# krrish94/nerf-pytorch

Hardware: AMD Instinct MI355X
Metric: train rays/sec (higher is better)
Workload: dtype f32

## Files before the change

### include/nerfhip.h

```cpp
#ifndef NERFHIP_H_
#define NERFHIP_H_

#include <stddef.h>
#include <stdint.h>

#ifdef __cplusplus
extern "C" {
#endif

typedef void* nerfhip_stream_t;

#define NERFHIP_OK 0
#define NERFHIP_ERR_ARG (-1)
#define NERFHIP_ERR_UNSUPPORTED (-2)
#define NERFHIP_ERR_LAUNCH (-3)
#define NERFHIP_ERR_WORKSPACE (-4)

#define NERFHIP_RNG_UNIFORM 0
#define NERFHIP_RNG_NORMAL 1

int nerfhip_version(void);
const char* nerfhip_last_error(void);
int nerfhip_is_emulated(void);

// ... 75 lines not shown
int nerfhip_plan_dim_xyz(nerfhip_plan_t plan);
int nerfhip_plan_dim_dir(nerfhip_plan_t plan);
int nerfhip_plan_num_tensors(nerfhip_plan_t plan);
int nerfhip_plan_tensor_info(nerfhip_plan_t plan, int i, const char** name, int64_t* offset, int* rows, int* cols);
int nerfhip_plan_describe(nerfhip_plan_t plan, char* buf, int64_t cap);
int64_t nerfhip_plan_packed_floats(nerfhip_plan_t plan);
int nerfhip_plan_pack_index(nerfhip_plan_t plan, int32_t* host_table);
int nerfhip_pack_weights(const float* params, const int32_t* table, int64_t n, float* packed, nerfhip_stream_t stream);
int nerfhip_pack_weights_plan(nerfhip_plan_t plan, const float* params, const int32_t* table, float* packed,
                              nerfhip_stream_t stream);
int64_t nerfhip_plan_stash_bytes(nerfhip_plan_t plan, int64_t m);
int64_t nerfhip_plan_bwd_scratch_bytes(nerfhip_plan_t plan, int64_t m);
int nerfhip_plan_set_bwd_compaction(nerfhip_plan_t plan, int on);
int nerfhip_plan_bwd_compaction(nerfhip_plan_t plan);
int64_t nerfhip_plan_bwd_stats_offset(nerfhip_plan_t plan, int64_t m);
int nerfhip_plan_set_freqs(nerfhip_plan_t plan, const float* freqs_xyz, const float* freqs_dir);

int nerfhip_mlp_fwd(nerfhip_plan_t plan, const float* packed, const float* x, int64_t m, float* out, void* stash,
                    nerfhip_stream_t stream);
int nerfhip_mlp_bwd(nerfhip_plan_t plan, const float* packed, const float* g_out, int64_t m, const void* stash,
                    void* scratch, int64_t scratch_bytes, float* g_params, nerfhip_stream_t stream);
int nerfhip_mlp_bwd_input(nerfhip_plan_t plan, const float* params, int64_t m, const void* scratch, float* g_x,
                          nerfhip_stream_t stream);

typedef struct nerfhip_render_cfg {
    int num_coarse;
    int num_fine;
    int perturb;
    int lindisp;
    int white_background;
// ... 250 lines not shown
```

### nerf-pytorch_amd/_lib.py

```python
import ctypes as C
import os

_HERE = os.path.dirname(os.path.abspath(__file__))
LIB_PATH = os.path.join(_HERE, "libnerfhip.so")

c_f = C.c_void_p
c_i64 = C.c_int64
c_u64 = C.c_uint64
c_u32 = C.c_uint32


class ModelCfg(C.Structure):
    _fields_ = [(n, C.c_int) for n in (
        "num_layers", "hidden_size", "skip_connect_every", "num_encoding_fn_xyz", "num_encoding_fn_dir",
        "include_input_xyz", "include_input_dir", "log_sampling_xyz", "log_sampling_dir", "use_viewdirs")]


class RenderCfg(C.Structure):
    _fields_ = [("num_coarse", C.c_int), ("num_fine", C.c_int), ("perturb", C.c_int), ("lindisp", C.c_int),
                ("white_background", C.c_int), ("noise_std", C.c_float), ("ray_stride", C.c_int)]


class RenderRand(C.Structure):
    _fields_ = [("t_rand", c_f), ("noise_coarse", c_f), ("u", c_f), ("noise_fine", c_f)]
# ... 72 lines not shown
    "nerfhip_plan_dim_xyz": (C.c_int, [C.c_void_p]),
    "nerfhip_plan_dim_dir": (C.c_int, [C.c_void_p]),
    "nerfhip_plan_num_tensors": (C.c_int, [C.c_void_p]),
    "nerfhip_plan_tensor_info": (C.c_int, [C.c_void_p, C.c_int, C.POINTER(C.c_char_p), C.POINTER(c_i64),
                                            C.POINTER(C.c_int), C.POINTER(C.c_int)]),
    "nerfhip_plan_packed_floats": (c_i64, [C.c_void_p]),
    "nerfhip_plan_describe": (C.c_int, [C.c_void_p, C.c_char_p, c_i64]),
    "nerfhip_plan_pack_index": (C.c_int, [C.c_void_p, C.c_void_p]),
    "nerfhip_pack_weights": (C.c_int, [c_f, c_f, c_i64, c_f, c_f]),
    "nerfhip_plan_stash_bytes": (c_i64, [C.c_void_p, c_i64]),
    "nerfhip_plan_bwd_scratch_bytes": (c_i64, [C.c_void_p, c_i64]),
    "nerfhip_plan_set_freqs": (C.c_int, [C.c_void_p, C.c_void_p, C.c_void_p]),
    "nerfhip_plan_set_bwd_compaction": (C.c_int, [C.c_void_p, C.c_int]),
    "nerfhip_plan_bwd_compaction": (C.c_int, [C.c_void_p]),
    "nerfhip_plan_bwd_stats_offset": (c_i64, [C.c_void_p, c_i64]),
    "nerfhip_mlp_fwd": (C.c_int, [C.c_void_p, c_f, c_f, c_i64, c_f, c_f, c_f]),
    "nerfhip_mlp_bwd": (C.c_int, [C.c_void_p, c_f, c_f, c_i64, c_f, c_f, c_i64, c_f, c_f]),
    "nerfhip_mlp_bwd_input": (C.c_int, [C.c_void_p, c_f, c_i64, c_f, c_f, c_f]),
    "nerfhip_render_workspace_bytes": (c_i64, [C.c_void_p, C.c_void_p, C.POINTER(RenderCfg), c_i64, C.c_int]),
    "nerfhip_render_workspace_region": (C.c_int, [C.c_void_p, C.c_void_p, C.POINTER(RenderCfg), c_i64, C.c_int, C.c_char_p,
                                                   C.POINTER(c_i64), C.POINTER(c_i64)]),
    "nerfhip_render_fwd": (C.c_int, [C.c_void_p, C.c_void_p, C.POINTER(RenderCfg), c_f, c_i64, c_f, c_f, c_f, c_f,
                                      C.POINTER(RenderRand), c_u64, c_u64, C.POINTER(RenderOut), c_f, c_i64, C.c_int,
                                      c_f]),
    "nerfhip_render_bwd": (C.c_int, [C.c_void_p, C.c_void_p, C.POINTER(RenderCfg), c_f, c_i64, c_f, c_f,
                                      C.POINTER(RenderRand), c_u64, c_u64, c_f, c_f, c_f, c_i64, c_f, c_f, c_f]),
    "nerfhip_render_fwd_parts": (C.c_int, [C.c_void_p, C.c_void_p, C.POINTER(RenderCfg), c_f, c_i64, c_f, c_f, c_f, c_f,
                                            C.POINTER(RenderRand), c_u64, c_u64, C.POINTER(RenderOut), c_f, c_i64,
                                            C.c_int, C.c_int, c_f]),
    "nerfhip_render_bwd_parts": (C.c_int, [C.c_void_p, C.c_void_p, C.POINTER(RenderCfg), c_f, c_i64, c_f, c_f,
# ... 163 lines not shown
```

### nerf-pytorch_amd/csrc/wgrad_f16.hip

```cpp
#include <vector>

#include "nh_device.h"
#include "nh_diag.h"
#include "nh_mlp.h"

namespace {

constexpr int NHW_MAX_JOBS = 40;
#ifndef NHW_WAVES
#define NHW_WAVES 8
#endif
constexpr int NHW_THREADS = 64 * NHW_WAVES;
#ifndef NHW_STAGES
#define NHW_STAGES 2
#endif

struct WgBJob {
    int64_t a_off, b_off;
    int wg0, nwg;
    int r_hi, col_count, w_ld;
    int64_t w_off, bias_off;
    int a_idx, b_idx;
    int64_t s_w_off;
    int s_w_ld;
};
struct WgBArgs {
    const float* stash;
    const float* grad;
    float* partial;
    float* g_params;
    int64_t nt;
    int njobs, part_stride;
    const unsigned* amax;
    const unsigned* bmax;
    int64_t s_off, s_bias_off;
    int s_idx, s_r_lo, s_r_hi, s_col_base, s_col_count;
    signed char scol[64];
    const int* cidx;
    const int* cstats;
    WgBJob jobs[NHW_MAX_JOBS];
};

NH_DEVICE int region_shift(unsigned word) { return word <= 1u ? 0 : 14 - ((int)word - 256); }
NH_DEVICE float unscale2(float v, int sa, int sb) { return (v * nh_pow2i(-sa)) * nh_pow2i(-sb); }

template <int AR, int BR, int SA = 0, int SB = 0>
struct WShape {
    static_assert(SA == 0 || SB == 0, "one guest per block");
    static_assert(NHW_WAVES == 8, "the side tiles are dealt to a 4 x 2 wave grid");
    static constexpr int PO = AR / (16 * NHW_WAVES), PI = BR / 64, TA = AR / 32, TB = BR / 32;
    static constexpr int SR = SA + SB;
    static constexpr int STAGE_A = AR * 64, STAGE_B = BR * 64, STAGE_S = SR * 64;
    static constexpr int STAGE = STAGE_A + STAGE_B + STAGE_S;
    static constexpr int OPER_A = AR * 32, OPER_B = BR * 32, OPER_S = SR * 32;
    static constexpr int LDS_BYTES = NHW_STAGES * STAGE + 2 * (OPER_A + OPER_B + OPER_S);
    static constexpr int SIDE_TILES = SB ? TA * (SB / 32) : (SA ? TB : 0);
    static constexpr int PART = AR * BR + SIDE_TILES * 1024 + NHW_THREADS + (SA ? 64 : 0);
};

template <int ROWS>
struct RowItems {
    static constexpr int N = (ROWS * 2 + NHW_THREADS - 1) / NHW_THREADS;
    float v[N][8];
};
template <int ROWS>
NH_DEVICE void rows_load(const float* stage, int tid, RowItems<ROWS>& r) {
#pragma unroll
    for (int it = 0; it < RowItems<ROWS>::N; ++it) {
        const int id = tid + NHW_THREADS * it;
        const bool on = ROWS * 2 % NHW_THREADS == 0 || id < ROWS * 2;
        const int row = id % ROWS, q = on ? id / ROWS : 0;
#pragma unroll
        for (int e = 0; e < 8; ++e) r.v[it][e] = on ? stage[(8 * q + e) * ROWS + row] : 0.0f;
    }
}
template <int ROWS>
NH_DEVICE float rows_store(const RowItems<ROWS>& r, char* hi_blocks, char* lo_blocks, int tid, float scale) {
    float sum = 0.0f;
#pragma unroll
    for (int it = 0; it < RowItems<ROWS>::N; ++it) {
        const int id = tid + NHW_THREADS * it;
        if (ROWS * 2 % NHW_THREADS != 0 && id >= ROWS * 2) break;
        const int row = id % ROWS, q = id / ROWS;
        nh_f16x8 h8, l8;
#pragma unroll
        for (int e = 0; e < 8; ++e) {
            float v = r.v[it][e];
            sum += v;
#ifdef NHW_EXP_NO_CONVERT
            h8[e] = nh_to_f16(v);
            l8[e] = h8[e];
            continue;
#endif
            v *= scale;
            const nh_f16 hi = nh_to_f16(v);
            h8[e] = hi;
            l8[e] = nh_to_f16(v - nh_from_f16(hi));
        }
        const int off = (((row >> 5) * 2 + q) * 32 + (row & 31)) * 16;
        *(nh_f16x8*)(hi_blocks + off) = h8;
        *(nh_f16x8*)(lo_blocks + off) = l8;
    }
    return sum;
// ... 17 lines not shown
        nh_dma16a(src, lane * 16, (int)(rows[0] * (unsigned)RB + ((unsigned)p * 1024u) % RB), lds_dst);
    } else {
        const int e = (lane * 16) / RB;
        unsigned row = rows[0];
#pragma unroll
        for (int k = 1; k < N; ++k) {
            row = e == k ? rows[k] : row;
#ifndef NERFHIP_EMU
            asm volatile("" : "+v"(row));
#endif
        }
        nh_dma16a(src, (int)(row * (unsigned)RB + (unsigned)(lane * 16) % RB), 0, lds_dst);
    }
}

template <int AR, int BR, int SA = 0, int SB = 0, bool CX = false>
NH_KERNEL void NH_LB(NHW_THREADS, NHW_WAVES / 4) k_wgrad_f16x3(WgBArgs a) {
    using S = WShape<AR, BR, SA, SB>;
    constexpr int PO = S::PO, PI = S::PI, SR = S::SR;
    NH_DYN_LDS(lds);
    char* const ah_blk = lds + NHW_STAGES * S::STAGE;
    char* const al_blk = ah_blk + S::OPER_A;
    char* const bh_blk = al_blk + S::OPER_A;
    char* const bl_blk = bh_blk + S::OPER_B;
    char* const sh_blk = bl_blk + S::OPER_B;
    char* const sl_blk = sh_blk + S::OPER_S;
    const int lane = nh_lane(), wave = nh_wave_in_block(), tid = (int)threadIdx.x;
    int jq = 0;
    while (jq + 1 < a.njobs && (int)blockIdx.x >= a.jobs[jq + 1].wg0) ++jq;
    const WgBJob& jb = a.jobs[jq];
    const int64_t k = (int64_t)blockIdx.x - jb.wg0;
    const int64_t ntl = CX ? (int64_t)((nh_uload_i32(a.cstats, NH_CSTAT_ACTIVE) + 31) >> 5) : a.nt;
    const int64_t u0 = 2 * (ntl * k / jb.nwg), u1 = 2 * (ntl * (k + 1) / jb.nwg);
    const float* const a_reg = a.grad + jb.a_off;
    const float* const b_reg = a.stash + jb.b_off;
    const float* const s_reg = SR ? (SA ? a.grad : a.stash) + a.s_off : nullptr;
    const float a_scale = a.amax ? nh_pow2i(region_shift(a.amax[jb.a_idx])) : 1.0f;
    const float b_scale = a.bmax ? nh_pow2i(region_shift(a.bmax[jb.b_idx])) : 1.0f;
    const float s_scale = (SR && a.amax && a.bmax) ? nh_pow2i(region_shift((SA ? a.amax : a.bmax)[a.s_idx])) : 1.0f;
    const unsigned lds0 = nh_lds_addr((const float*)lds);
    constexpr int PIECES = (S::STAGE_A + S::STAGE_B) / (1024 * NHW_WAVES);
    constexpr int SPIECES = S::STAGE_S / 1024;
    static_assert(S::STAGE_A % (1024 * NHW_WAVES) == 0 && S::STAGE_B % (1024 * NHW_WAVES) == 0, "every wave issues the same number of pieces");
    static_assert(SPIECES <= NHW_WAVES, "at most one side piece per wave");
    constexpr int NPB = S::STAGE_B / 1024 / NHW_WAVES;
    static_assert(!CX || NPB * NHW_WAVES * 1024 == S::STAGE_B, "every wave gathers the same number of B pieces");
    unsigned rb[NPB * GatherN<BR>::N > 0 ? NPB * GatherN<BR>::N : 1], rs[GatherN<(SB ? SB : 32)>::N];
    auto preload = [&](int64_t u) {
        if (CX && a.cidx) {
#pragma unroll
            for (int j = 0; j < NPB; ++j) gather_rows<BR>(rb + j * GatherN<BR>::N, a.cidx, (int)u * 16, wave + j * NHW_WAVES);
            if (SB) gather_rows<(SB ? SB : 32)>(rs, a.cidx, (int)u * 16, wave < SPIECES ? wave : 0);
        }
    };
    auto issue = [&](int64_t u) {
        const NhDmaSrc da = nh_dma_src(a_reg + (size_t)u * 16 * AR, (unsigned)S::STAGE_A);
        const unsigned st = lds0 + (unsigned)((int)(u % NHW_STAGES) * S::STAGE);
        for (int p = wave; p < S::STAGE_A / 1024; p += NHW_WAVES) nh_dma16a(da, lane * 16, p * 1024, st + (unsigned)(p * 1024));
        if (CX && a.cidx) {
            const NhDmaSrc db = nh_dma_src(b_reg, (unsigned)((size_t)a.nt * 32 * BR * 4));
#pragma unroll
            for (int j = 0; j < NPB; ++j)
                gather_piece_f16<BR>(db, rb + j * GatherN<BR>::N, wave + j * NHW_WAVES, lane, st + (unsigned)(S::STAGE_A + (wave + j * NHW_WAVES) * 1024));
        } else {
            const NhDmaSrc db = nh_dma_src(b_reg + (size_t)u * 16 * BR, (unsigned)S::STAGE_B);
            for (int p = wave; p < S::STAGE_B / 1024; p += NHW_WAVES) nh_dma16a(db, lane * 16, p * 1024, st + (unsigned)(S::STAGE_A + p * 1024));
        }
        if (SR) {
            if (CX && SB && a.cidx) {
                const NhDmaSrc ds = nh_dma_src(s_reg, (unsigned)((size_t)a.nt * 32 * (SR ? SR : 1) * 4));
// ... 8 lines not shown
#pragma unroll
    for (int x = 0; x < PO; ++x)
#pragma unroll
        for (int y = 0; y < PI; ++y)
#pragma unroll
            for (int c = 0; c < 16; ++c) acc[x][y][c] = 0.0f;
    constexpr int NSACC = SB ? PO : (SA ? 1 : 1);
    f32x16 sacc[NSACC];
#pragma unroll
    for (int x = 0; x < NSACC; ++x)
#pragma unroll
        for (int c = 0; c < 16; ++c) sacc[x][c] = 0.0f;
    const int wo = wave >> 1, wi = wave & 1;
    const bool side_on = SB ? (SB == 64 || wi == 0) : (SA ? wo < PI : false);
    const int ys = wo % PI;
    float bias = 0.0f, sbias = 0.0f;
    const int ta0 = wo * PO, tb0 = wi * PI;
#pragma unroll
    for (int d = 0; d < NHW_STAGES; ++d)
        if (u0 + d < u1) {
            preload(u0 + d);
            issue(u0 + d);
        }
    for (int64_t u = u0; u < u1; ++u) {
        if (u + NHW_STAGES < u1) preload(u + NHW_STAGES);
#ifndef NHW_EXP_NO_WAIT
        const int64_t behind = u1 - 1 - u < NHW_STAGES - 1 ? u1 - 1 - u : NHW_STAGES - 1;
        if (behind >= 2) {
            if (wave < SPIECES) nh_wait_vmem_keep<2 * (PIECES + 1)>();
            else nh_wait_vmem_keep<2 * PIECES>();
        } else if (behind == 1) {
            if (wave < SPIECES) nh_wait_vmem_keep<PIECES + 1>();
            else nh_wait_vmem_keep<PIECES>();
        } else {
            nh_wait_vmem();
        }
#endif
        nh_block_sync();
        const char* const stage = lds + (int)(u % NHW_STAGES) * S::STAGE;
        RowItems<AR> ra;
        RowItems<BR> rb;
        RowItems<(SR ? SR : 32)> rs;
// ... 51 lines not shown
#pragma unroll
                for (int x = 0; x < PO; ++x) sacc[x] = nh_mfma_f16(ah[x], sh, sacc[x]);
            }
        } else if (SA) {
            if (side_on) {
#pragma unroll
                for (int y = 0; y < PI; ++y)
                    if (y == ys) {
                        sacc[0] = nh_mfma_f16(sl, bh[y], sacc[0]);
                        sacc[0] = nh_mfma_f16(sh, bl[y], sacc[0]);
                        sacc[0] = nh_mfma_f16(sh, bh[y], sacc[0]);
                    }
            }
        }
    }
    float* const part = a.partial + (size_t)blockIdx.x * (size_t)a.part_stride;
#pragma unroll
    for (int x = 0; x < PO; ++x)
#pragma unroll
        for (int y = 0; y < PI; ++y)
#pragma unroll
            for (int c = 0; c < 16; ++c) part[((ta0 + x) * S::TB + (tb0 + y)) * 1024 + c * 64 + lane] = acc[x][y][c];
    if (SB) {
        if (side_on) {
            const int st = SB == 64 ? wi : 0;
#pragma unroll
            for (int x = 0; x < PO; ++x)
#pragma unroll
                for (int c = 0; c < 16; ++c) part[AR * BR + ((ta0 + x) * (SB / 32) + st) * 1024 + c * 64 + lane] = sacc[x][c];
        }
    } else if (SA) {
        if (side_on) {
#pragma unroll
            for (int c = 0; c < 16; ++c) part[AR * BR + (tb0 + ys) * 1024 + c * 64 + lane] = sacc[0][c];
        }
    }
    part[AR * BR + S::SIDE_TILES * 1024 + tid] = bias;
    if (SA && tid < 64) part[AR * BR + S::SIDE_TILES * 1024 + NHW_THREADS + tid] = sbias;
}

template <int AR, int BR, int SA = 0, int SB = 0>
NH_KERNEL void k_wgrad_reduce_f16x3(WgBArgs a) {
    using S = WShape<AR, BR, SA, SB>;
    constexpr int TB = BR / 32, E = AR * BR, SE = S::SIDE_TILES * 1024, NALL = E + AR + SE + SA, GX = (NALL + 255) / 256;
    const int jq = (int)blockIdx.x / GX;
    const WgBJob& jb = a.jobs[jq];
    const int e = ((int)blockIdx.x % GX) * 256 + (int)threadIdx.x;
    const bool scaled = a.amax && a.bmax;
    auto sum_partials = [&](int64_t off) {
        float s8[8] = {0.f, 0.f, 0.f, 0.f, 0.f, 0.f, 0.f, 0.f};
        const float* const src = a.partial + (size_t)jb.wg0 * (size_t)a.part_stride + off;
        int k = 0;
        for (; k + 8 <= jb.nwg; k += 8) {
#pragma unroll
            for (int q = 0; q < 8; ++q) s8[q] += src[(size_t)(k + q) * (size_t)a.part_stride];
        }
        for (int q = 0; k < jb.nwg; ++k, ++q) s8[q] += src[(size_t)k * (size_t)a.part_stride];
        return ((s8[0] + s8[1]) + (s8[2] + s8[3])) + ((s8[4] + s8[5]) + (s8[6] + s8[7]));
    };
    if (e < E) {
        const int tile = e >> 10, c = (e >> 6) & 15, l = e & 63;
        const int row = 32 * (tile / TB) + (c & 3) + 8 * (c >> 2) + 4 * (l >> 5), col = 32 * (tile % TB) + (l & 31);
        if (row < jb.r_hi && col < jb.col_count) {
            const float v = sum_partials(e);
            a.g_params[jb.w_off + (int64_t)row * jb.w_ld + col] = scaled ? unscale2(v, region_shift(a.amax[jb.a_idx]), region_shift(a.bmax[jb.b_idx])) : v;
        }
    } else if (e < E + AR) {
        const int row = e - E;
        if (row < jb.r_hi && jb.bias_off >= 0) {
            float s8[8] = {0.f, 0.f, 0.f, 0.f, 0.f, 0.f, 0.f, 0.f};
            const float* const src = a.partial + (size_t)jb.wg0 * (size_t)a.part_stride + E + SE + row;
            int k = 0;
            for (; k + 8 <= jb.nwg; k += 8) {
#pragma unroll
                for (int q = 0; q < 8; ++q)
#pragma unroll
                    for (int t = 0; t < NHW_THREADS; t += AR) s8[q] += src[(size_t)(k + q) * (size_t)a.part_stride + t];
            }
            for (int q = 0; k < jb.nwg; ++k, ++q)
#pragma unroll
                for (int t = 0; t < NHW_THREADS; t += AR) s8[q] += src[(size_t)k * (size_t)a.part_stride + t];
            a.g_params[jb.bias_off + row] = ((s8[0] + s8[1]) + (s8[2] + s8[3])) + ((s8[4] + s8[5]) + (s8[6] + s8[7]));
        }
    } else if (e < E + AR + SE) {
        const int se = e - E - AR, tile = se >> 10, c = (se >> 6) & 15, l = se & 63;
        const int r32 = (c & 3) + 8 * (c >> 2) + 4 * (l >> 5);
        if (SB) {
            const int row = 32 * (tile / (SB / 32)) + r32, slot = 32 * (tile % (SB / 32)) + (l & 31);
            const int col = (int)a.scol[slot];
            if (row < jb.r_hi && col >= 0 && col < a.s_col_count) {
                const float v = sum_partials(E + se);
                a.g_params[jb.s_w_off + (int64_t)row * jb.s_w_ld + a.s_col_base + col] =
                    scaled ? unscale2(v, region_shift(a.amax[jb.a_idx]), region_shift(a.bmax[a.s_idx])) : v;
            }
        } else {
            const int col = 32 * tile + (l & 31);
            if (r32 >= a.s_r_lo && r32 < a.s_r_hi && col < jb.col_count) {
                const float v = sum_partials(E + se);
                a.g_params[jb.s_w_off + (int64_t)(r32 - a.s_r_lo) * jb.s_w_ld + col] =
                    scaled ? unscale2(v, region_shift(a.amax[a.s_idx]), region_shift(a.bmax[jb.b_idx])) : v;
            }
        }
    } else if (SA && e < NALL) {
        const int r = e - E - AR - SE;
        if (r >= a.s_r_lo && r < a.s_r_hi && a.s_bias_off >= 0)
            a.g_params[a.s_bias_off + (r - a.s_r_lo)] = sum_partials(E + SE + NHW_THREADS + r) + sum_partials(E + SE + NHW_THREADS + SA + r);
    }
}

#ifndef NHW_WGS
#define NHW_WGS 768
#endif
#ifndef NHW_WGS_HALF
#define NHW_WGS_HALF 256
#endif

struct LaunchB {
    int ar, sa, sb;
    WgBArgs w;
};

int64_t schedule(nerfhip_plan* p, int64_t nt, std::vector<LaunchB>* out) {
    const int W = p->W;
    std::vector<LaunchB> L;
    std::vector<char> side_set;
    for (const NhJobB& j : p->bjobs) {
        const int sa = j.side_kind == 1 ? j.side_rows : 0, sb = j.side_kind == 2 ? j.side_rows : 0;
        size_t q = 0;
        while (q < L.size() && !(L[q].ar == j.a_rows && L[q].sa == sa && L[q].sb == sb)) ++q;
        if (q == L.size()) {
            LaunchB l;
            memset(&l, 0, sizeof(l));
            l.ar = j.a_rows, l.sa = sa, l.sb = sb;
            l.w.s_bias_off = -1;
            for (int k = 0; k < 64; ++k) l.w.scol[k] = -1;
            L.push_back(l);
            side_set.push_back(0);
        }
        WgBArgs& w = L[q].w;
        if (w.njobs >= NHW_MAX_JOBS) {
            nh_set_error("wgrad_f16: more than %d blocks of one shape in a launch", NHW_MAX_JOBS);
            return -1;
        }
        WgBJob& d = w.jobs[w.njobs++];
        d.a_off = 32 * nt * j.a_row_prefix;
        d.b_off = 32 * nt * j.b_row_prefix;
        d.r_hi = j.r_hi;
        d.col_count = j.col_count;
        d.w_ld = j.w_ld;
        d.w_off = j.w_off;
        d.bias_off = j.bias_off;
        d.a_idx = j.a_idx;
        d.b_idx = j.b_idx;
        d.s_w_off = j.s_w_off;
        d.s_w_ld = j.s_w_ld;
        if (j.side_kind) {
            const int64_t s_off = 32 * nt * j.side_row_prefix;
            const bool first = !side_set[q];
            if (!first && (w.s_off != s_off || w.s_idx != j.side_idx || w.s_r_lo != j.s_r_lo || w.s_r_hi != j.s_r_hi ||
                           w.s_col_base != j.s_col_base || w.s_col_count != j.s_col_count ||
                           (j.s_bias_off >= 0 && w.s_bias_off >= 0 && w.s_bias_off != j.s_bias_off))) {
                nh_set_error("wgrad_f16: two guest regions of one shape in a launch (rows %d, side rows %d / %d)", j.a_rows, sa, sb);
                return -1;
            }
            side_set[q] = true;
            w.s_off = s_off;
            w.s_idx = j.side_idx;
            w.s_r_lo = j.s_r_lo;
            w.s_r_hi = j.s_r_hi;
            w.s_col_base = j.s_col_base;
            w.s_col_count = j.s_col_count;
            if (j.s_bias_off >= 0) w.s_bias_off = j.s_bias_off;
            const int* map = j.s_col_kind == 1 ? p->xyz_slot_col : p->dir_slot_col;
            if (j.side_kind == 2)
                for (int k = 0; k < j.side_rows && k < 64; ++k) w.scol[k] = (signed char)map[k];
        }
    }
    int64_t floats = 0;
    for (LaunchB& l : L) {
        WgBArgs& w = l.w;
        const bool plain_full = l.ar == W && !l.sa && !l.sb;
        int64_t nwg = (plain_full ? NHW_WGS / w.njobs : NHW_WGS_HALF);
        if (nwg < 1) nwg = 1;
        if (nwg > nt) nwg = nt > 0 ? nt : 1;
        int wg = 0;
        for (int q = 0; q < w.njobs; ++q) {
            w.jobs[q].wg0 = wg;
            w.jobs[q].nwg = (int)nwg;
            wg += (int)nwg;
        }
        const int side_tiles = l.sb ? (l.ar / 32) * (l.sb / 32) : (l.sa ? W / 32 : 0);
        w.part_stride = l.ar * W + side_tiles * 1024 + NHW_THREADS + (l.sa ? 64 : 0);
        w.nt = nt;
        floats += (int64_t)wg * w.part_stride;
    }
    if (out) *out = L;
    return floats;
}

template <int AR, int BR, int SA, int SB>
int launch(WgBArgs& w, nerfhip_stream_t stream) {
    if (w.njobs == 0) return NERFHIP_OK;
    using S = WShape<AR, BR, SA, SB>;
    static_assert(S::PART == AR * BR + S::SIDE_TILES * 1024 + NHW_THREADS + (SA ? 64 : 0), "schedule() sizes the partials");
    const int wgs = w.jobs[w.njobs - 1].wg0 + w.jobs[w.njobs - 1].nwg;
    int rc = NERFHIP_OK;
    if (w.cstats) {
        rc = nh_lds_limit(k_wgrad_f16x3<AR, BR, SA, SB, true>, S::LDS_BYTES);
        if (rc) return rc;
        NH_LAUNCH_NAMED(AR == BR ? (SA || SB ? "k_wgrad_f16x3<full+side, compacted>" : "k_wgrad_f16x3<full, compacted>")
                                 : (SA || SB ? "k_wgrad_f16x3<half+side, compacted>" : "k_wgrad_f16x3<half, compacted>"),
                        (k_wgrad_f16x3<AR, BR, SA, SB, true>), wgs, NHW_THREADS, (S::LDS_BYTES), stream, w);
    } else {
        rc = nh_lds_limit(k_wgrad_f16x3<AR, BR, SA, SB>, S::LDS_BYTES);
        if (rc) return rc;
        NH_LAUNCH_NAMED(AR == BR ? (SA || SB ? "k_wgrad_f16x3<full+side>" : "k_wgrad_f16x3<full>")
                                 : (SA || SB ? "k_wgrad_f16x3<half+side>" : "k_wgrad_f16x3<half>"),
                        (k_wgrad_f16x3<AR, BR, SA, SB>), wgs, NHW_THREADS, (S::LDS_BYTES), stream, w);
    }
    rc = nh_launch_status("wgrad_f16x3");
    if (rc) return rc;
    constexpr int NALL = AR * BR + AR + S::SIDE_TILES * 1024 + SA;
    NH_LAUNCH_NAMED("k_wgrad_f16_reduce", (k_wgrad_reduce_f16x3<AR, BR, SA, SB>), ((NALL + 255) / 256) * w.njobs, 256, 0, stream, w);
    return nh_launch_status("wgrad_f16_reduce");
}

}

int64_t nh_wgrad_x3_partial_floats(nerfhip_plan* p, int64_t nt) {
    if (p->bjobs.empty()) return 0;
    return schedule(p, nt > 0 ? nt : 1, nullptr);
}

int nh_wgrad_f16(nerfhip_plan* p, int64_t nt, const float* stash, const float* grad, float* partial, float* g_params,
                 const unsigned* amax, const unsigned* bmax, const NhCompact* cx, nerfhip_stream_t stream) {
    if (p->bjobs.empty()) return NERFHIP_OK;
    NH_REQUIRE((int)p->bjobs.size() <= NHW_MAX_JOBS, "wgrad_f16: too many blocks");
    std::vector<LaunchB> L;
    if (schedule(p, nt, &L) < 0) return NERFHIP_ERR_UNSUPPORTED;
    int rc = NERFHIP_OK;
    int64_t off = 0;
    for (LaunchB& l : L) {
        WgBArgs& w = l.w;
        w.stash = stash;
        w.grad = grad;
        w.g_params = g_params;
        w.amax = amax;
        w.bmax = bmax;
        w.cidx = (cx && !cx->stash_in_list_order) ? cx->idx : nullptr;
        w.cstats = cx ? cx->stats : nullptr;
        w.partial = partial + off;
        off += (int64_t)(w.jobs[w.njobs - 1].wg0 + w.jobs[w.njobs - 1].nwg) * w.part_stride;
        const int W = p->W;
        if (W == 256 && l.ar == 256 && !l.sa && !l.sb) rc = launch<256, 256, 0, 0>(w, stream);
        else if (W == 256 && l.ar == 256 && l.sb == 64) rc = launch<256, 256, 0, 64>(w, stream);
        else if (W == 256 && l.ar == 256 && l.sa == 32) rc = launch<256, 256, 32, 0>(w, stream);
        else if (W == 256 && l.ar == 128 && !l.sa && !l.sb) rc = launch<128, 256, 0, 0>(w, stream);
        else if (W == 256 && l.ar == 128 && l.sb == 32) rc = launch<128, 256, 0, 32>(w, stream);
        else if (W == 128 && l.ar == 128 && !l.sa && !l.sb) rc = launch<128, 128, 0, 0>(w, stream);
        else if (W == 128 && l.ar == 128 && l.sb == 64) rc = launch<128, 128, 0, 64>(w, stream);
        else if (W == 128 && l.ar == 128 && l.sa == 32) rc = launch<128, 128, 32, 0>(w, stream);
        else {
            nh_set_error("wgrad_f16: no kernel for kernel width %d, %d-row blocks with side rows %d / %d", W, l.ar, l.sa, l.sb);
            return NERFHIP_ERR_UNSUPPORTED;
        }
        if (rc) return rc;
    }
    return rc;
}
```

Before: 150,000.

## Merge all f16 wgrad block shapes into one cost-balanced launch

```diff
diff --git a/include/nerfhip.h b/include/nerfhip.h
--- a/include/nerfhip.h
+++ b/include/nerfhip.h
@@ -113,6 +113,8 @@
 int nerfhip_plan_set_bwd_compaction(nerfhip_plan_t plan, int on);
 int nerfhip_plan_bwd_compaction(nerfhip_plan_t plan);
 int64_t nerfhip_plan_bwd_stats_offset(nerfhip_plan_t plan, int64_t m);
+int64_t nerfhip_plan_wgrad_f16_schedule(nerfhip_plan_t plan, int64_t n_tiles, int64_t* out, int64_t cap, int64_t* partial_floats,
+                                        int64_t* wg_limit);
 int nerfhip_plan_set_freqs(nerfhip_plan_t plan, const float* freqs_xyz, const float* freqs_dir);
 
 int nerfhip_mlp_fwd(nerfhip_plan_t plan, const float* packed, const float* x, int64_t m, float* out, void* stash,
diff --git a/nerf-pytorch_amd/_lib.py b/nerf-pytorch_amd/_lib.py
--- a/nerf-pytorch_amd/_lib.py
+++ b/nerf-pytorch_amd/_lib.py
@@ -110,6 +110,7 @@
     "nerfhip_plan_set_bwd_compaction": (C.c_int, [C.c_void_p, C.c_int]),
     "nerfhip_plan_bwd_compaction": (C.c_int, [C.c_void_p]),
     "nerfhip_plan_bwd_stats_offset": (c_i64, [C.c_void_p, c_i64]),
+    "nerfhip_plan_wgrad_f16_schedule": (c_i64, [C.c_void_p, c_i64, C.c_void_p, c_i64, C.c_void_p, C.c_void_p]),
     "nerfhip_mlp_fwd": (C.c_int, [C.c_void_p, c_f, c_f, c_i64, c_f, c_f, c_f]),
     "nerfhip_mlp_bwd": (C.c_int, [C.c_void_p, c_f, c_f, c_i64, c_f, c_f, c_i64, c_f, c_f]),
     "nerfhip_mlp_bwd_input": (C.c_int, [C.c_void_p, c_f, c_i64, c_f, c_f, c_f]),
diff --git a/nerf-pytorch_amd/csrc/wgrad_f16.hip b/nerf-pytorch_amd/csrc/wgrad_f16.hip
--- a/nerf-pytorch_amd/csrc/wgrad_f16.hip
+++ b/nerf-pytorch_amd/csrc/wgrad_f16.hip
@@ -1,4 +1,3 @@
-#include <vector>
 
 #include "nh_device.h"
 #include "nh_diag.h"
@@ -15,14 +14,18 @@
 #define NHW_STAGES 2
 #endif
 
+enum { NHW_FULL = 0, NHW_FULL_SB64 = 1, NHW_FULL_SA32 = 2, NHW_HALF = 3, NHW_HALF_SB32 = 4 };
+
 struct WgBJob {
     int64_t a_off, b_off;
+    int64_t w_off, bias_off;
+    int64_t part_off;
+    int64_t s_off, s_w_off, s_bias_off;
     int wg0, nwg;
-    int r_hi, col_count, w_ld;
-    int64_t w_off, bias_off;
-    int a_idx, b_idx;
-    int64_t s_w_off;
-    int s_w_ld;
+    int rg0;
+    short r_hi, col_count, w_ld, s_w_ld, s_col_base, s_col_count;
+    unsigned char a_idx, b_idx, s_idx;
+    unsigned char shape, s_map, s_r_lo, s_r_hi;
 };
 struct WgBArgs {
     const float* stash;
@@ -30,16 +33,15 @@
     float* partial;
     float* g_params;
     int64_t nt;
-    int njobs, part_stride;
+    int njobs;
     const unsigned* amax;
     const unsigned* bmax;
-    int64_t s_off, s_bias_off;
-    int s_idx, s_r_lo, s_r_hi, s_col_base, s_col_count;
-    signed char scol[64];
+    signed char xcol[64], dcol[64];
     const int* cidx;
     const int* cstats;
     WgBJob jobs[NHW_MAX_JOBS];
 };
+static_assert(sizeof(WgBArgs) <= 4096, "the kernel arguments travel by value: 4 KB at most");
 
 NH_DEVICE int region_shift(unsigned word) { return word <= 1u ? 0 : 14 - ((int)word - 256); }
 NH_DEVICE float unscale2(float v, int sa, int sb) { return (v * nh_pow2i(-sa)) * nh_pow2i(-sb); }
@@ -55,7 +57,8 @@
     static constexpr int OPER_A = AR * 32, OPER_B = BR * 32, OPER_S = SR * 32;
     static constexpr int LDS_BYTES = NHW_STAGES * STAGE + 2 * (OPER_A + OPER_B + OPER_S);
     static constexpr int SIDE_TILES = SB ? TA * (SB / 32) : (SA ? TB : 0);
-    static constexpr int PART = AR * BR + SIDE_TILES * 1024 + NHW_THREADS + (SA ? 64 : 0);
+    static constexpr int PART = AR * BR + SIDE_TILES * 1024 + 2 * NHW_THREADS + (SA ? 128 : 0);
+    static constexpr int NALL = AR * BR + AR + SIDE_TILES * 1024 + SA;
 };
 
 template <int ROWS>
@@ -75,8 +78,8 @@
     }
 }
 template <int ROWS>
-NH_DEVICE float rows_store(const RowItems<ROWS>& r, char* hi_blocks, char* lo_blocks, int tid, float scale) {
-    float sum = 0.0f;
+NH_DEVICE double rows_store(const RowItems<ROWS>& r, char* hi_blocks, char* lo_blocks, int tid, float scale) {
+    double sum = 0.0;
 #pragma unroll
     for (int it = 0; it < RowItems<ROWS>::N; ++it) {
         const int id = tid + NHW_THREADS * it;
@@ -86,7 +89,7 @@
 #pragma unroll
         for (int e = 0; e < 8; ++e) {
             float v = r.v[it][e];
-            sum += v;
+            sum += (double)v;
 #ifdef NHW_EXP_NO_CONVERT
             h8[e] = nh_to_f16(v);
             l8[e] = h8[e];
@@ -134,8 +137,17 @@
     }
 }
 
-template <int AR, int BR, int SA = 0, int SB = 0, bool CX = false>
-NH_KERNEL void NH_LB(NHW_THREADS, NHW_WAVES / 4) k_wgrad_f16x3(WgBArgs a) {
+template <bool CX>
+struct StepOf {
+    typedef int64_t type;
+};
+template <>
+struct StepOf<true> {
+    typedef int type;
+};
+
+template <int AR, int BR, int SA, int SB, bool CX>
+NH_DEVICE void wgrad_f16x3_block(const WgBArgs& a, const WgBJob& jb) {
     using S = WShape<AR, BR, SA, SB>;
     constexpr int PO = S::PO, PI = S::PI, SR = S::SR;
     NH_DYN_LDS(lds);
@@ -146,18 +158,16 @@
     char* const sh_blk = bl_blk + S::OPER_B;
     char* const sl_blk = sh_blk + S::OPER_S;
     const int lane = nh_lane(), wave = nh_wave_in_block(), tid = (int)threadIdx.x;
-    int jq = 0;
-    while (jq + 1 < a.njobs && (int)blockIdx.x >= a.jobs[jq + 1].wg0) ++jq;
-    const WgBJob& jb = a.jobs[jq];
     const int64_t k = (int64_t)blockIdx.x - jb.wg0;
     const int64_t ntl = CX ? (int64_t)((nh_uload_i32(a.cstats, NH_CSTAT_ACTIVE) + 31) >> 5) : a.nt;
-    const int64_t u0 = 2 * (ntl * k / jb.nwg), u1 = 2 * (ntl * (k + 1) / jb.nwg);
+    typedef typename StepOf<CX>::type step_t;
+    const step_t u0 = (step_t)(2 * (ntl * k / jb.nwg)), u1 = (step_t)(2 * (ntl * (k + 1) / jb.nwg));
     const float* const a_reg = a.grad + jb.a_off;
     const float* const b_reg = a.stash + jb.b_off;
-    const float* const s_reg = SR ? (SA ? a.grad : a.stash) + a.s_off : nullptr;
+    const float* const s_reg = SR ? (SA ? a.grad : a.stash) + jb.s_off : nullptr;
     const float a_scale = a.amax ? nh_pow2i(region_shift(a.amax[jb.a_idx])) : 1.0f;
     const float b_scale = a.bmax ? nh_pow2i(region_shift(a.bmax[jb.b_idx])) : 1.0f;
-    const float s_scale = (SR && a.amax && a.bmax) ? nh_pow2i(region_shift((SA ? a.amax : a.bmax)[a.s_idx])) : 1.0f;
+    const float s_scale = (SR && a.amax && a.bmax) ? nh_pow2i(region_shift((SA ? a.amax : a.bmax)[jb.s_idx])) : 1.0f;
     const unsigned lds0 = nh_lds_addr((const float*)lds);
     constexpr int PIECES = (S::STAGE_A + S::STAGE_B) / (1024 * NHW_WAVES);
     constexpr int SPIECES = S::STAGE_S / 1024;
@@ -166,14 +176,14 @@
     constexpr int NPB = S::STAGE_B / 1024 / NHW_WAVES;
     static_assert(!CX || NPB * NHW_WAVES * 1024 == S::STAGE_B, "every wave gathers the same number of B pieces");
     unsigned rb[NPB * GatherN<BR>::N > 0 ? NPB * GatherN<BR>::N : 1], rs[GatherN<(SB ? SB : 32)>::N];
-    auto preload = [&](int64_t u) {
+    auto preload = [&](step_t u) {
         if (CX && a.cidx) {
 #pragma unroll
             for (int j = 0; j < NPB; ++j) gather_rows<BR>(rb + j * GatherN<BR>::N, a.cidx, (int)u * 16, wave + j * NHW_WAVES);
             if (SB) gather_rows<(SB ? SB : 32)>(rs, a.cidx, (int)u * 16, wave < SPIECES ? wave : 0);
         }
     };
-    auto issue = [&](int64_t u) {
+    auto issue = [&](step_t u) {
         const NhDmaSrc da = nh_dma_src(a_reg + (size_t)u * 16 * AR, (unsigned)S::STAGE_A);
         const unsigned st = lds0 + (unsigned)((int)(u % NHW_STAGES) * S::STAGE);
         for (int p = wave; p < S::STAGE_A / 1024; p += NHW_WAVES) nh_dma16a(da, lane * 16, p * 1024, st + (unsigned)(p * 1024));
@@ -212,7 +222,7 @@
     const int wo = wave >> 1, wi = wave & 1;
     const bool side_on = SB ? (SB == 64 || wi == 0) : (SA ? wo < PI : false);
     const int ys = wo % PI;
-    float bias = 0.0f, sbias = 0.0f;
+    double bias = 0.0, sbias = 0.0;
     const int ta0 = wo * PO, tb0 = wi * PI;
 #pragma unroll
     for (int d = 0; d < NHW_STAGES; ++d)
@@ -220,10 +230,10 @@
             preload(u0 + d);
             issue(u0 + d);
         }
-    for (int64_t u = u0; u < u1; ++u) {
+    for (step_t u = u0; u < u1; ++u) {
         if (u + NHW_STAGES < u1) preload(u + NHW_STAGES);
 #ifndef NHW_EXP_NO_WAIT
-        const int64_t behind = u1 - 1 - u < NHW_STAGES - 1 ? u1 - 1 - u : NHW_STAGES - 1;
+        const step_t behind = u1 - 1 - u < NHW_STAGES - 1 ? u1 - 1 - u : NHW_STAGES - 1;
         if (behind >= 2) {
             if (wave < SPIECES) nh_wait_vmem_keep<2 * (PIECES + 1)>();
             else nh_wait_vmem_keep<2 * PIECES>();
@@ -305,7 +315,7 @@
             }
         }
     }
-    float* const part = a.partial + (size_t)blockIdx.x * (size_t)a.part_stride;
+    float* const part = a.partial + jb.part_off + k * S::PART;
 #pragma unroll
     for (int x = 0; x < PO; ++x)
 #pragma unroll
@@ -326,27 +336,49 @@
             for (int c = 0; c < 16; ++c) part[AR * BR + (tb0 + ys) * 1024 + c * 64 + lane] = sacc[0][c];
         }
     }
-    part[AR * BR + S::SIDE_TILES * 1024 + tid] = bias;
-    if (SA && tid < 64) part[AR * BR + S::SIDE_TILES * 1024 + NHW_THREADS + tid] = sbias;
-}
-
-template <int AR, int BR, int SA = 0, int SB = 0>
-NH_KERNEL void k_wgrad_reduce_f16x3(WgBArgs a) {
+    float* const pb = part + AR * BR + S::SIDE_TILES * 1024;
+    pb[tid] = (float)bias;
+    pb[NHW_THREADS + tid] = (float)(bias - (double)(float)bias);
+    if (SA && tid < 64) {
+        pb[2 * NHW_THREADS + tid] = (float)sbias;
+        pb[2 * NHW_THREADS + 64 + tid] = (float)(sbias - (double)(float)sbias);
+    }
+}
+
+template <int W, bool CX>
+NH_KERNEL void NH_LB(NHW_THREADS, NHW_WAVES / 4) k_wgrad_f16x3(WgBArgs a) {
+    int jq = 0;
+    while (jq + 1 < a.njobs && (int)blockIdx.x >= a.jobs[jq + 1].wg0) ++jq;
+    const WgBJob& jb = a.jobs[jq];
+    const int shape = (int)jb.shape;
+    if (shape == NHW_FULL) {
+        wgrad_f16x3_block<W, W, 0, 0, CX>(a, jb);
+    } else if (shape == NHW_FULL_SB64) {
+        wgrad_f16x3_block<W, W, 0, 64, CX>(a, jb);
+    } else if (shape == NHW_FULL_SA32) {
+        wgrad_f16x3_block<W, W, 32, 0, CX>(a, jb);
+    } else if constexpr (W == 256) {
+        if (shape == NHW_HALF) wgrad_f16x3_block<128, 256, 0, 0, CX>(a, jb);
+        else wgrad_f16x3_block<128, 256, 0, 32, CX>(a, jb);
+    }
+}
+
+template <int AR, int BR, int SA, int SB>
+NH_DEVICE void wgrad_f16x3_reduce_block(const WgBArgs& a, const WgBJob& jb, int e) {
     using S = WShape<AR, BR, SA, SB>;
-    constexpr int TB = BR / 32, E = AR * BR, SE = S::SIDE_TILES * 1024, NALL = E + AR + SE + SA, GX = (NALL + 255) / 256;
-    const int jq = (int)blockIdx.x / GX;
-    const WgBJob& jb = a.jobs[jq];
-    const int e = ((int)blockIdx.x % GX) * 256 + (int)threadIdx.x;
+    constexpr int TB = BR / 32, E = AR * BR, SE = S::SIDE_TILES * 1024, NALL = S::NALL;
+    constexpr size_t PART = (size_t)S::PART;
     const bool scaled = a.amax && a.bmax;
+    const float* const part0 = a.partial + jb.part_off;
     auto sum_partials = [&](int64_t off) {
         float s8[8] = {0.f, 0.f, 0.f, 0.f, 0.f, 0.f, 0.f, 0.f};
-        const float* const src = a.partial + (size_t)jb.wg0 * (size_t)a.part_stride + off;
+        const float* const src = part0 + off;
         int k = 0;
         for (; k + 8 <= jb.nwg; k += 8) {
 #pragma unroll
-            for (int q = 0; q < 8; ++q) s8[q] += src[(size_t)(k + q) * (size_t)a.part_stride];
-        }
-        for (int q = 0; k < jb.nwg; ++k, ++q) s8[q] += src[(size_t)k * (size_t)a.part_stride];
+            for (int q = 0; q < 8; ++q) s8[q] += src[(size_t)(k + q) * PART];
+        }
+        for (int q = 0; k < jb.nwg; ++k, ++q) s8[q] += src[(size_t)k * PART];
         return ((s8[0] + s8[1]) + (s8[2] + s8[3])) + ((s8[4] + s8[5]) + (s8[6] + s8[7]));
     };
     if (e < E) {
@@ -359,160 +391,252 @@
     } else if (e < E + AR) {
         const int row = e - E;
         if (row < jb.r_hi && jb.bias_off >= 0) {
-            float s8[8] = {0.f, 0.f, 0.f, 0.f, 0.f, 0.f, 0.f, 0.f};
-            const float* const src = a.partial + (size_t)jb.wg0 * (size_t)a.part_stride + E + SE + row;
+            double s8[8] = {0., 0., 0., 0., 0., 0., 0., 0.};
+            const float* const src = part0 + E + SE + row;
             int k = 0;
             for (; k + 8 <= jb.nwg; k += 8) {
 #pragma unroll
                 for (int q = 0; q < 8; ++q)
 #pragma unroll
-                    for (int t = 0; t < NHW_THREADS; t += AR) s8[q] += src[(size_t)(k + q) * (size_t)a.part_stride + t];
+                    for (int t = 0; t < NHW_THREADS; t += AR)
+                        s8[q] += (double)src[(size_t)(k + q) * PART + t] + (double)src[(size_t)(k + q) * PART + NHW_THREADS + t];
             }
             for (int q = 0; k < jb.nwg; ++k, ++q)
 #pragma unroll
-                for (int t = 0; t < NHW_THREADS; t += AR) s8[q] += src[(size_t)k * (size_t)a.part_stride + t];
-            a.g_params[jb.bias_off + row] = ((s8[0] + s8[1]) + (s8[2] + s8[3])) + ((s8[4] + s8[5]) + (s8[6] + s8[7]));
+                for (int t = 0; t < NHW_THREADS; t += AR) s8[q] += (double)src[(size_t)k * PART + t] + (double)src[(size_t)k * PART + NHW_THREADS + t];
+            a.g_params[jb.bias_off + row] = (float)(((s8[0] + s8[1]) + (s8[2] + s8[3])) + ((s8[4] + s8[5]) + (s8[6] + s8[7])));
         }
     } else if (e < E + AR + SE) {
         const int se = e - E - AR, tile = se >> 10, c = (se >> 6) & 15, l = se & 63;
         const int r32 = (c & 3) + 8 * (c >> 2) + 4 * (l >> 5);
         if (SB) {
             const int row = 32 * (tile / (SB / 32)) + r32, slot = 32 * (tile % (SB / 32)) + (l & 31);
-            const int col = (int)a.scol[slot];
-            if (row < jb.r_hi && col >= 0 && col < a.s_col_count) {
+            const int col = (int)(jb.s_map == 1 ? a.xcol : a.dcol)[slot];
+            if (row < jb.r_hi && col >= 0 && col < jb.s_col_count) {
                 const float v = sum_partials(E + se);
-                a.g_params[jb.s_w_off + (int64_t)row * jb.s_w_ld + a.s_col_base + col] =
-                    scaled ? unscale2(v, region_shift(a.amax[jb.a_idx]), region_shift(a.bmax[a.s_idx])) : v;
+                a.g_params[jb.s_w_off + (int64_t)row * jb.s_w_ld + jb.s_col_base + col] =
+                    scaled ? unscale2(v, region_shift(a.amax[jb.a_idx]), region_shift(a.bmax[jb.s_idx])) : v;
             }
         } else {
             const int col = 32 * tile + (l & 31);
-            if (r32 >= a.s_r_lo && r32 < a.s_r_hi && col < jb.col_count) {
+            if (r32 >= jb.s_r_lo && r32 < jb.s_r_hi && col < jb.col_count) {
                 const float v = sum_partials(E + se);
-                a.g_params[jb.s_w_off + (int64_t)(r32 - a.s_r_lo) * jb.s_w_ld + col] =
-                    scaled ? unscale2(v, region_shift(a.amax[a.s_idx]), region_shift(a.bmax[jb.b_idx])) : v;
+                a.g_params[jb.s_w_off + (int64_t)(r32 - jb.s_r_lo) * jb.s_w_ld + col] =
+                    scaled ? unscale2(v, region_shift(a.amax[jb.s_idx]), region_shift(a.bmax[jb.b_idx])) : v;
             }
         }
     } else if (SA && e < NALL) {
         const int r = e - E - AR - SE;
-        if (r >= a.s_r_lo && r < a.s_r_hi && a.s_bias_off >= 0)
-            a.g_params[a.s_bias_off + (r - a.s_r_lo)] = sum_partials(E + SE + NHW_THREADS + r) + sum_partials(E + SE + NHW_THREADS + SA + r);
-    }
-}
-
-#ifndef NHW_WGS
-#define NHW_WGS 768
+        if (r >= jb.s_r_lo && r < jb.s_r_hi && jb.s_bias_off >= 0) {
+            double s8[8] = {0., 0., 0., 0., 0., 0., 0., 0.};
+            const float* const src = part0 + E + SE + 2 * NHW_THREADS + r;
+            int k = 0;
+            for (; k + 8 <= jb.nwg; k += 8) {
+#pragma unroll
+                for (int q = 0; q < 8; ++q) {
+                    const float* const w = src + (size_t)(k + q) * PART;
+                    s8[q] += ((double)w[0] + (double)w[64]) + ((double)w[SA] + (double)w[64 + SA]);
+                }
+            }
+            for (int q = 0; k < jb.nwg; ++k, ++q) {
+                const float* const w = src + (size_t)k * PART;
+                s8[q] += ((double)w[0] + (double)w[64]) + ((double)w[SA] + (double)w[64 + SA]);
+            }
+            a.g_params[jb.s_bias_off + (r - jb.s_r_lo)] = (float)(((s8[0] + s8[1]) + (s8[2] + s8[3])) + ((s8[4] + s8[5]) + (s8[6] + s8[7])));
+        }
+    }
+}
+
+template <int W>
+NH_KERNEL void k_wgrad_reduce_f16x3(WgBArgs a) {
+    int jq = 0;
+    while (jq + 1 < a.njobs && (int)blockIdx.x >= a.jobs[jq + 1].rg0) ++jq;
+    const WgBJob& jb = a.jobs[jq];
+    const int e = ((int)blockIdx.x - jb.rg0) * 256 + (int)threadIdx.x;
+    const int shape = (int)jb.shape;
+    if (shape == NHW_FULL) {
+        wgrad_f16x3_reduce_block<W, W, 0, 0>(a, jb, e);
+    } else if (shape == NHW_FULL_SB64) {
+        wgrad_f16x3_reduce_block<W, W, 0, 64>(a, jb, e);
+    } else if (shape == NHW_FULL_SA32) {
+        wgrad_f16x3_reduce_block<W, W, 32, 0>(a, jb, e);
+    } else if constexpr (W == 256) {
+        if (shape == NHW_HALF) wgrad_f16x3_reduce_block<128, 256, 0, 0>(a, jb, e);
+        else wgrad_f16x3_reduce_block<128, 256, 0, 32>(a, jb, e);
+    }
+}
+
+#ifndef NHW_ROUNDS
+#define NHW_ROUNDS 1
 #endif
-#ifndef NHW_WGS_HALF
-#define NHW_WGS_HALF 256
-#endif
-
-struct LaunchB {
-    int ar, sa, sb;
+constexpr int NHW_WG_LIMIT = NHW_ROUNDS * 256;
+constexpr int NHW_GUEST_COST_PCT = 124;
+
+struct ShapeDims {
+    int part, nall, lds;
+};
+template <int AR, int BR, int SA, int SB>
+constexpr ShapeDims shape_dims_of() {
+    using S = WShape<AR, BR, SA, SB>;
+    return ShapeDims{S::PART, S::NALL, S::LDS_BYTES};
+}
+int shape_of(int W, int ar, int sa, int sb) {
+    if (W != 128 && W != 256) return -1;
+    if (ar == W && !sa && !sb) return NHW_FULL;
+    if (ar == W && !sa && sb == 64) return NHW_FULL_SB64;
+    if (ar == W && sa == 32 && !sb) return NHW_FULL_SA32;
+    if (W == 256 && ar == 128 && !sa && !sb) return NHW_HALF;
+    if (W == 256 && ar == 128 && !sa && sb == 32) return NHW_HALF_SB32;
+    return -1;
+}
+ShapeDims shape_dims(int W, int shape) {
+    if (W == 256) {
+        switch (shape) {
+            case NHW_FULL: return shape_dims_of<256, 256, 0, 0>();
+            case NHW_FULL_SB64: return shape_dims_of<256, 256, 0, 64>();
+            case NHW_FULL_SA32: return shape_dims_of<256, 256, 32, 0>();
+            case NHW_HALF: return shape_dims_of<128, 256, 0, 0>();
+            default: return shape_dims_of<128, 256, 0, 32>();
+        }
+    }
+    switch (shape) {
+        case NHW_FULL: return shape_dims_of<128, 128, 0, 0>();
+        case NHW_FULL_SB64: return shape_dims_of<128, 128, 0, 64>();
+        default: return shape_dims_of<128, 128, 32, 0>();
+    }
+}
+
+struct Sched {
     WgBArgs w;
-};
-
-int64_t schedule(nerfhip_plan* p, int64_t nt, std::vector<LaunchB>* out) {
+    int wgs, rgs, lds;
+    int part[NHW_MAX_JOBS];
+    int64_t floats;
+};
+
+int64_t schedule(nerfhip_plan* p, int64_t nt, Sched* s) {
     const int W = p->W;
-    std::vector<LaunchB> L;
-    std::vector<char> side_set;
+    memset(s, 0, sizeof(*s));
+    WgBArgs& w = s->w;
+    for (int k = 0; k < 64; ++k) w.xcol[k] = w.dcol[k] = -1;
+    if ((int)p->bjobs.size() > NHW_MAX_JOBS) {
+        nh_set_error("wgrad_f16: more than %d blocks in a launch", NHW_MAX_JOBS);
+        return -1;
+    }
+    int64_t cost[NHW_MAX_JOBS], cost_sum = 0;
     for (const NhJobB& j : p->bjobs) {
         const int sa = j.side_kind == 1 ? j.side_rows : 0, sb = j.side_kind == 2 ? j.side_rows : 0;
-        size_t q = 0;
-        while (q < L.size() && !(L[q].ar == j.a_rows && L[q].sa == sa && L[q].sb == sb)) ++q;
-        if (q == L.size()) {
-            LaunchB l;
-            memset(&l, 0, sizeof(l));
-            l.ar = j.a_rows, l.sa = sa, l.sb = sb;
-            l.w.s_bias_off = -1;
-            for (int k = 0; k < 64; ++k) l.w.scol[k] = -1;
-            L.push_back(l);
-            side_set.push_back(0);
-        }
-        WgBArgs& w = L[q].w;
-        if (w.njobs >= NHW_MAX_JOBS) {
-            nh_set_error("wgrad_f16: more than %d blocks of one shape in a launch", NHW_MAX_JOBS);
+        const int shape = shape_of(W, j.a_rows, sa, sb);
+        if (shape < 0 || j.b_rows != W) {
+            nh_set_error("wgrad_f16: no kernel for kernel width %d, %d-row blocks with side rows %d / %d", W, j.a_rows, sa, sb);
             return -1;
         }
-        WgBJob& d = w.jobs[w.njobs++];
+        const int vals[] = {j.r_hi, j.col_count, j.w_ld, j.s_w_ld, j.s_col_base, j.s_col_count};
+        for (int v : vals)
+            if (v < 0 || v > 32767) {
+                nh_set_error("wgrad_f16: a block's row / column count %d does not fit its table entry", v);
+                return -1;
+            }
+        if (j.a_idx < 0 || j.a_idx > 255 || j.b_idx < 0 || j.b_idx > 255 || j.side_idx < 0 || j.side_idx > 255 || j.s_r_lo < 0 ||
+            j.s_r_hi > 255 || j.s_r_lo > j.s_r_hi) {
+            nh_set_error("wgrad_f16: a block's region slot or side rows do not fit its table entry");
+            return -1;
+        }
+        const int q = w.njobs++;
+        WgBJob& d = w.jobs[q];
+        d.shape = (unsigned char)shape;
         d.a_off = 32 * nt * j.a_row_prefix;
         d.b_off = 32 * nt * j.b_row_prefix;
-        d.r_hi = j.r_hi;
-        d.col_count = j.col_count;
-        d.w_ld = j.w_ld;
+        d.r_hi = (short)j.r_hi;
+        d.col_count = (short)j.col_count;
+        d.w_ld = (short)j.w_ld;
         d.w_off = j.w_off;
         d.bias_off = j.bias_off;
-        d.a_idx = j.a_idx;
-        d.b_idx = j.b_idx;
+        d.a_idx = (unsigned char)j.a_idx;
+        d.b_idx = (unsigned char)j.b_idx;
         d.s_w_off = j.s_w_off;
-        d.s_w_ld = j.s_w_ld;
+        d.s_w_ld = (short)j.s_w_ld;
+        d.s_bias_off = -1;
         if (j.side_kind) {
-            const int64_t s_off = 32 * nt * j.side_row_prefix;
-            const bool first = !side_set[q];
-            if (!first && (w.s_off != s_off || w.s_idx != j.side_idx || w.s_r_lo != j.s_r_lo || w.s_r_hi != j.s_r_hi ||
-                           w.s_col_base != j.s_col_base || w.s_col_count != j.s_col_count ||
-                           (j.s_bias_off >= 0 && w.s_bias_off >= 0 && w.s_bias_off != j.s_bias_off))) {
-                nh_set_error("wgrad_f16: two guest regions of one shape in a launch (rows %d, side rows %d / %d)", j.a_rows, sa, sb);
-                return -1;
-            }
-            side_set[q] = true;
-            w.s_off = s_off;
-            w.s_idx = j.side_idx;
-            w.s_r_lo = j.s_r_lo;
-            w.s_r_hi = j.s_r_hi;
-            w.s_col_base = j.s_col_base;
-            w.s_col_count = j.s_col_count;
-            if (j.s_bias_off >= 0) w.s_bias_off = j.s_bias_off;
-            const int* map = j.s_col_kind == 1 ? p->xyz_slot_col : p->dir_slot_col;
-            if (j.side_kind == 2)
-                for (int k = 0; k < j.side_rows && k < 64; ++k) w.scol[k] = (signed char)map[k];
-        }
-    }
+            d.s_off = 32 * nt * j.side_row_prefix;
+            d.s_idx = (unsigned char)j.side_idx;
+            d.s_r_lo = (unsigned char)j.s_r_lo;
+            d.s_r_hi = (unsigned char)j.s_r_hi;
+            d.s_col_base = (short)j.s_col_base;
+            d.s_col_count = (short)j.s_col_count;
+            d.s_bias_off = j.s_bias_off;
+            d.s_map = (unsigned char)j.s_col_kind;
+            if (j.side_kind == 2) {
+                const int* map = j.s_col_kind == 1 ? p->xyz_slot_col : p->dir_slot_col;
+                signed char* col = j.s_col_kind == 1 ? w.xcol : w.dcol;
+                for (int k = 0; k < j.side_rows && k < 64; ++k) col[k] = (signed char)map[k];
+            }
+        }
+        cost[q] = (int64_t)(j.a_rows + j.b_rows + j.side_rows) * 128 * (j.side_kind ? NHW_GUEST_COST_PCT : 100);
+        cost_sum += cost[q];
+        const ShapeDims dm = shape_dims(W, shape);
+        s->part[q] = dm.part;
+        if (dm.lds > s->lds) s->lds = dm.lds;
+        d.rg0 = s->rgs;
+        s->rgs += (dm.nall + 255) / 256;
+    }
+    const int n = w.njobs;
+    if (n == 0) return 0;
+    const int64_t cap = nt > 0 ? nt : 1;
+    int64_t nwg[NHW_MAX_JOBS], rem[NHW_MAX_JOBS], given = 0;
+    for (int q = 0; q < n; ++q) {
+        nwg[q] = NHW_WG_LIMIT * cost[q] / cost_sum;
+        rem[q] = NHW_WG_LIMIT * cost[q] % cost_sum;
+        given += nwg[q];
+    }
+    for (; given < NHW_WG_LIMIT; ++given) {
+        int best = 0;
+        for (int q = 1; q < n; ++q)
+            if (rem[q] > rem[best]) best = q;
+        ++nwg[best];
+        rem[best] = -1;
+    }
+    int64_t total = 0;
+    for (int q = 0; q < n; ++q) {
+        nwg[q] = nwg[q] < 1 ? 1 : (nwg[q] > cap ? cap : nwg[q]);
+        total += nwg[q];
+    }
+    for (; total > NHW_WG_LIMIT; --total) {
+        int best = 0;
+        for (int q = 1; q < n; ++q)
+            if (nwg[q] > nwg[best]) best = q;
+        --nwg[best];
+    }
+    int wg = 0;
     int64_t floats = 0;
-    for (LaunchB& l : L) {
-        WgBArgs& w = l.w;
-        const bool plain_full = l.ar == W && !l.sa && !l.sb;
-        int64_t nwg = (plain_full ? NHW_WGS / w.njobs : NHW_WGS_HALF);
-        if (nwg < 1) nwg = 1;
-        if (nwg > nt) nwg = nt > 0 ? nt : 1;
-        int wg = 0;
-        for (int q = 0; q < w.njobs; ++q) {
-            w.jobs[q].wg0 = wg;
-            w.jobs[q].nwg = (int)nwg;
-            wg += (int)nwg;
-        }
-        const int side_tiles = l.sb ? (l.ar / 32) * (l.sb / 32) : (l.sa ? W / 32 : 0);
-        w.part_stride = l.ar * W + side_tiles * 1024 + NHW_THREADS + (l.sa ? 64 : 0);
-        w.nt = nt;
-        floats += (int64_t)wg * w.part_stride;
-    }
-    if (out) *out = L;
+    for (int q = 0; q < n; ++q) {
+        w.jobs[q].wg0 = wg;
+        w.jobs[q].nwg = (int)nwg[q];
+        w.jobs[q].part_off = floats;
+        wg += (int)nwg[q];
+        floats += nwg[q] * s->part[q];
+    }
+    w.nt = nt;
+    s->wgs = wg;
+    s->floats = floats;
     return floats;
 }
 
-template <int AR, int BR, int SA, int SB>
-int launch(WgBArgs& w, nerfhip_stream_t stream) {
-    if (w.njobs == 0) return NERFHIP_OK;
-    using S = WShape<AR, BR, SA, SB>;
-    static_assert(S::PART == AR * BR + S::SIDE_TILES * 1024 + NHW_THREADS + (SA ? 64 : 0), "schedule() sizes the partials");
-    const int wgs = w.jobs[w.njobs - 1].wg0 + w.jobs[w.njobs - 1].nwg;
+template <int W>
+int launch(Sched& s, nerfhip_stream_t stream) {
+    WgBArgs& w = s.w;
     int rc = NERFHIP_OK;
     if (w.cstats) {
-        rc = nh_lds_limit(k_wgrad_f16x3<AR, BR, SA, SB, true>, S::LDS_BYTES);
+        rc = nh_lds_limit(k_wgrad_f16x3<W, true>, s.lds);
         if (rc) return rc;
-        NH_LAUNCH_NAMED(AR == BR ? (SA || SB ? "k_wgrad_f16x3<full+side, compacted>" : "k_wgrad_f16x3<full, compacted>")
-                                 : (SA || SB ? "k_wgrad_f16x3<half+side, compacted>" : "k_wgrad_f16x3<half, compacted>"),
-                        (k_wgrad_f16x3<AR, BR, SA, SB, true>), wgs, NHW_THREADS, (S::LDS_BYTES), stream, w);
+        NH_LAUNCH_NAMED("k_wgrad_f16x3<all, compacted>", (k_wgrad_f16x3<W, true>), s.wgs, NHW_THREADS, s.lds, stream, w);
     } else {
-        rc = nh_lds_limit(k_wgrad_f16x3<AR, BR, SA, SB>, S::LDS_BYTES);
+        rc = nh_lds_limit(k_wgrad_f16x3<W, false>, s.lds);
         if (rc) return rc;
-        NH_LAUNCH_NAMED(AR == BR ? (SA || SB ? "k_wgrad_f16x3<full+side>" : "k_wgrad_f16x3<full>")
-                                 : (SA || SB ? "k_wgrad_f16x3<half+side>" : "k_wgrad_f16x3<half>"),
-                        (k_wgrad_f16x3<AR, BR, SA, SB>), wgs, NHW_THREADS, (S::LDS_BYTES), stream, w);
+        NH_LAUNCH_NAMED("k_wgrad_f16x3<all>", (k_wgrad_f16x3<W, false>), s.wgs, NHW_THREADS, s.lds, stream, w);
     }
     rc = nh_launch_status("wgrad_f16x3");
     if (rc) return rc;
-    constexpr int NALL = AR * BR + AR + S::SIDE_TILES * 1024 + SA;
-    NH_LAUNCH_NAMED("k_wgrad_f16_reduce", (k_wgrad_reduce_f16x3<AR, BR, SA, SB>), ((NALL + 255) / 256) * w.njobs, 256, 0, stream, w);
+    NH_LAUNCH_NAMED("k_wgrad_f16_reduce", (k_wgrad_reduce_f16x3<W>), s.rgs, 256, 0, stream, w);
     return nh_launch_status("wgrad_f16_reduce");
 }
 
@@ -520,42 +644,42 @@
 
 int64_t nh_wgrad_x3_partial_floats(nerfhip_plan* p, int64_t nt) {
     if (p->bjobs.empty()) return 0;
-    return schedule(p, nt > 0 ? nt : 1, nullptr);
+    Sched s;
+    return schedule(p, nt > 0 ? nt : 1, &s);
+}
+
+extern "C" int64_t nerfhip_plan_wgrad_f16_schedule(nerfhip_plan_t plan, int64_t n_tiles, int64_t* out, int64_t cap, int64_t* partial_floats,
+                                                   int64_t* wg_limit) {
+    if (!plan || n_tiles < 1 || (cap > 0 && !out)) {
+        nh_set_error("plan_wgrad_f16_schedule: bad arguments");
+        return -1;
+    }
+    Sched s;
+    if (schedule(plan, n_tiles, &s) < 0) return -1;
+    for (int q = 0; q < s.w.njobs && q < cap; ++q) {
+        out[4 * q + 0] = s.w.jobs[q].wg0;
+        out[4 * q + 1] = s.w.jobs[q].nwg;
+        out[4 * q + 2] = s.part[q];
+        out[4 * q + 3] = s.w.jobs[q].part_off;
+    }
+    if (partial_floats) *partial_floats = s.floats;
+    if (wg_limit) *wg_limit = NHW_WG_LIMIT;
+    return s.w.njobs;
 }
 
 int nh_wgrad_f16(nerfhip_plan* p, int64_t nt, const float* stash, const float* grad, float* partial, float* g_params,
                  const unsigned* amax, const unsigned* bmax, const NhCompact* cx, nerfhip_stream_t stream) {
     if (p->bjobs.empty()) return NERFHIP_OK;
-    NH_REQUIRE((int)p->bjobs.size() <= NHW_MAX_JOBS, "wgrad_f16: too many blocks");
-    std::vector<LaunchB> L;
-    if (schedule(p, nt, &L) < 0) return NERFHIP_ERR_UNSUPPORTED;
-    int rc = NERFHIP_OK;
-    int64_t off = 0;
-    for (LaunchB& l : L) {
-        WgBArgs& w = l.w;
-        w.stash = stash;
-        w.grad = grad;
-        w.g_params = g_params;
-        w.amax = amax;
-        w.bmax = bmax;
-        w.cidx = (cx && !cx->stash_in_list_order) ? cx->idx : nullptr;
-        w.cstats = cx ? cx->stats : nullptr;
-        w.partial = partial + off;
-        off += (int64_t)(w.jobs[w.njobs - 1].wg0 + w.jobs[w.njobs - 1].nwg) * w.part_stride;
-        const int W = p->W;
-        if (W == 256 && l.ar == 256 && !l.sa && !l.sb) rc = launch<256, 256, 0, 0>(w, stream);
-        else if (W == 256 && l.ar == 256 && l.sb == 64) rc = launch<256, 256, 0, 64>(w, stream);
-        else if (W == 256 && l.ar == 256 && l.sa == 32) rc = launch<256, 256, 32, 0>(w, stream);
-        else if (W == 256 && l.ar == 128 && !l.sa && !l.sb) rc = launch<128, 256, 0, 0>(w, stream);
-        else if (W == 256 && l.ar == 128 && l.sb == 32) rc = launch<128, 256, 0, 32>(w, stream);
-        else if (W == 128 && l.ar == 128 && !l.sa && !l.sb) rc = launch<128, 128, 0, 0>(w, stream);
-        else if (W == 128 && l.ar == 128 && l.sb == 64) rc = launch<128, 128, 0, 64>(w, stream);
-        else if (W == 128 && l.ar == 128 && l.sa == 32) rc = launch<128, 128, 32, 0>(w, stream);
-        else {
-            nh_set_error("wgrad_f16: no kernel for kernel width %d, %d-row blocks with side rows %d / %d", W, l.ar, l.sa, l.sb);
-            return NERFHIP_ERR_UNSUPPORTED;
-        }
-        if (rc) return rc;
-    }
-    return rc;
-}
+    Sched s;
+    if (schedule(p, nt, &s) < 0) return NERFHIP_ERR_UNSUPPORTED;
+    WgBArgs& w = s.w;
+    w.stash = stash;
+    w.grad = grad;
+    w.partial = partial;
+    w.g_params = g_params;
+    w.amax = amax;
+    w.bmax = bmax;
+    w.cidx = (cx && !cx->stash_in_list_order) ? cx->idx : nullptr;
+    w.cstats = cx ? cx->stats : nullptr;
+    return p->W == 256 ? launch<256>(s, stream) : launch<128>(s, stream);
+}
```

Result: no change. 149,800 (-0.1%).
